# l90lpa/fv3-jedi-linearmodel

Measured on AMD Instinct MI355X. Metric: column-updates/s per TL+AD dyn step, higher is better.
Workload: dtype f64; 1 GPU; C192L127 hydrostatic TL+AD, six cube faces dealt over 1 GPU(s) (6 per rank), table-driven exchange (221184 columns per GPU), k_split=2 n_split=6 dt=450s nq=4, hord mt/vt/tm/dp/tr=2/2/2/2/2 (sponge: 1/1/1/1 below level 9), kord=17, nord=1; columns_per_gpu=221184

## Files before the change

fv3_jedi_linearmodel_amd/csrc/dycore.h:

```cpp
#pragma once
#include "../../include/fv3lm.h"
#include "stages.h"
#include "column.h"
#include "exchange.h"
#include "nh.h"
#include "nh_ad.h"
#include "tpfused.h"
#include "tpad.h"
#include "tp2.h"
#include "dampt.h"
#include "dext.h"
#include "a2b.h"
#include "d2a2c.h"
#include "del6.h"
#include <functional>
#include <map>
#include <memory>
#include <set>
#include <string>
#include <vector>

namespace fv3 {

#ifdef FV3LM_HOST_EMUL
inline void* dev_alloc(size_t n) { void* p = std::calloc(n ? n : 1, 1); return p; }
inline void dev_free(void* p) { std::free(p); }
inline void dev_zero(Exec&, void* p, size_t n) { std::memset(p, 0, n); }
inline void dev_copy(Exec&, void* d, const void* s, size_t n) { std::memcpy(d, s, n); }
inline void h2d(Exec&, void* d, const void* s, size_t n) { std::memcpy(d, s, n); }
inline void d2h(Exec&, void* d, const void* s, size_t n) { std::memcpy(d, s, n); }
inline void dev_sync(Exec&) {}
#else
#define HIPCHK(x) do { hipError_t e_ = (x); if (e_ != hipSuccess) { char b_[320]; std::snprintf(b_, sizeof b_, "HIP error '%s' at %s:%d (%s)", hipGetErrorString(e_), __FILE__, __LINE__, #x); set_sticky(b_); } } while (0)
inline void* dev_alloc(size_t n) {
  void* p = nullptr;
  if (!sticky_error().empty()) return nullptr;
  const hipError_t e = hipMalloc(&p, n ? n : 8);
  if (e != hipSuccess) { char b_[200]; std::snprintf(b_, sizeof b_, "hipMalloc of %zu bytes failed: %s", n, hipGetErrorString(e)); set_sticky(b_); (void)hipGetLastError(); return nullptr; }
  HIPCHK(hipMemset(p, 0, n ? n : 8));
  return p;
}
inline void dev_free(void* p) { if (p) (void)hipFree(p); }
__global__ void __launch_bounds__(256) k_zero16(double2* p, size_t n2) {
  const size_t stride = (size_t)gridDim.x * 256;
  for (size_t i = (size_t)blockIdx.x * 256 + threadIdx.x; i < n2; i += stride) p[i] = make_double2(0., 0.);
}
inline void dev_zero(Exec& ex, void* p, size_t n) {
  if (n >= ((size_t)1 << 20) && ((uintptr_t)p & 7) == 0) {
    char* q = (char*)p;
    if ((uintptr_t)q & 15) { HIPCHK(hipMemsetAsync(q, 0, 8, ex.stream)); q += 8; n -= 8; }
    const size_t n2 = n / 16, want = (n2 + 255) / 256;
    hipLaunchKernelGGL(k_zero16, dim3((unsigned)(want < 8192 ? want : 8192)), dim3(256), 0, ex.stream, (double2*)q, n2);
    if (n & 15) HIPCHK(hipMemsetAsync(q + n2 * 16, 0, n & 15, ex.stream));
    return;
  }
  HIPCHK(hipMemsetAsync(p, 0, n, ex.stream));
}
inline void dev_copy(Exec& ex, void* d, const void* s, size_t n) { HIPCHK(hipMemcpyAsync(d, s, n, hipMemcpyDeviceToDevice, ex.stream)); }
inline void h2d(Exec& ex, void* d, const void* s, size_t n) { HIPCHK(hipMemcpyAsync(d, s, n, hipMemcpyHostToDevice, ex.stream)); HIPCHK(hipStreamSynchronize(ex.stream)); }
inline void d2h(Exec& ex, void* d, const void* s, size_t n) { HIPCHK(hipMemcpyAsync(d, s, n, hipMemcpyDeviceToHost, ex.stream)); HIPCHK(hipStreamSynchronize(ex.stream)); }
inline void dev_sync(Exec& ex) { HIPCHK(hipStreamSynchronize(ex.stream)); }
#endif

struct Arena {
  double* t = nullptr; double* p = nullptr; size_t cap = 0, used = 0;
  void measure() { cap = (size_t)1 << 56; t = p = (double*)(uintptr_t)4096; used = 0; }
  void init(size_t ndoubles) { cap = ndoubles; t = (double*)dev_alloc(cap * 8); p = (double*)dev_alloc(cap * 8); used = 0; }
  void destroy() { dev_free(t); dev_free(p); t = p = nullptr; }
  Fld take(size_t n, int nk) {
    if (used + n > cap) { set_sticky("internal sizing error: field arena overflow"); Fld f; f.t = t; f.p = p; f.nk = nk; return f; }
    Fld f; f.t = t + used; f.p = p + used; f.nk = nk; used += n; return f;
  }
};

struct CkSet {
  struct Item { std::string name; double* p; size_t n, off; };
  std::string name; std::vector<Item> items; size_t stride = 0; int nrec = 0; double* buf = nullptr;
  void add(const std::string& nm, double* p, size_t ndoubles) { items.push_back(Item{nm, p, ndoubles, stride}); stride += ndoubles; }
  void add(const std::string& nm, const Fld& f, size_t plane) { add(nm, f.t, (size_t)f.nk * plane); }
  void alloc(const char* nm, int nrec_) {
    name = nm; buf = nrec_ > 0 ? (double*)dev_alloc(stride * nrec_ * 8) : nullptr; nrec = buf ? nrec_ : 0;
    if (std::getenv("FV3LM_VERBOSE")) std::fprintf(stderr, "fv3lm: checkpoint set %s: %d records, %zu bytes\n", nm, nrec, stride * nrec * 8);
  }
  void destroy() { dev_free(buf); buf = nullptr; nrec = 0; }
  int item(const char* nm) const {
    for (int n = 0; n < (int)items.size(); ++n) if (items[(size_t)n].name == nm) return n;
    set_sticky("internal error: checkpoint set " + name + " has no item " + nm); return -1;
  }
  size_t bytes(int item) const { return items[(size_t)item].n * 8; }
  double* at(int rec, int item) const {
    if (buf && rec >= 0 && rec < nrec && item >= 0 && item < (int)items.size()) return buf + (size_t)rec * stride + items[(size_t)item].off;
    set_sticky("internal error: checkpoint set " + name + ": record " + std::to_string(rec) + " item " + std::to_string(item) + " out of range"); return nullptr;
  }
  void save(Exec& ex, int rec, int item) const { if (double* q_ = at(rec, item)) dev_copy(ex, q_, items[(size_t)item].p, bytes(item)); }
  void restore(Exec& ex, int rec, int item, double* to = nullptr) const {
    if (const double* q_ = at(rec, item)) dev_copy(ex, to ? to : items[(size_t)item].p, q_, bytes(item));
  }
  void save(Exec& ex, int rec) const { for (int n = 0; n < (int)items.size(); ++n) save(ex, rec, n); }
  void restore(Exec& ex, int rec) const { for (int n = 0; n < (int)items.size(); ++n) restore(ex, rec, n); }
  void redirect(Exec& ex, int rec, int item, const double* from) const { if (double* q_ = at(rec, item)) ex.redirect_t(from, q_); }
};

typedef fv3lm_options Options;

inline bool resolve_level(const Options& o, int k, int npz, LevelParams& lp) {
  int hord_m = o.hord_mt, hord_t = o.hord_tm, hord_v = o.hord_vt, hord_p = o.hord_dp;
  int nord_k = o.nord, nord_v = (2 > o.nord) ? o.nord : 2;
  double d2_divg = (0.20 > o.d2_bg) ? o.d2_bg : 0.20;
  double damp_vt = o.do_vort_damp ? o.vtdm4 : 0.;
  int nord_w = nord_v, nord_t = nord_v;
  double damp_w = damp_vt, damp_t = damp_vt, d_con_k = o.d_con;
  if (npz == 1 || o.n_sponge < 0) {
    d2_divg = o.d2_bg;
  } else if (k == 1) {
    nord_k = 0;
    if (0.01 < o.d2_bg) d2_divg = (o.d2_bg < o.d2_bg_k1) ? o.d2_bg_k1 : o.d2_bg;
    else if (0.01 < o.d2_bg_k1) d2_divg = o.d2_bg_k1;
    else d2_divg = 0.01;
    nord_w = 0; damp_w = d2_divg;
    if (o.do_vort_damp) { nord_v = 0; damp_vt = 0.5 * d2_divg; }
    d_con_k = 0.;
  } else {
    const int max1 = (2 < o.n_sponge - 1) ? o.n_sponge - 1 : 2;
    if (k == max1 && o.d2_bg_k2 > 0.01) {
      nord_k = 0; d2_divg = (o.d2_bg < o.d2_bg_k2) ? o.d2_bg_k2 : o.d2_bg;
      nord_w = 0; damp_w = d2_divg;
      if (o.do_vort_damp) { nord_v = 0; damp_vt = 0.5 * d2_divg; }
      d_con_k = 0.;
    } else {
      const int max2 = (3 < o.n_sponge) ? o.n_sponge : 3;
      if (k == max2 && o.d2_bg_k2 > 0.05) {
        nord_k = 0; d2_divg = (o.d2_bg < 0.2 * o.d2_bg_k2) ? 0.2 * o.d2_bg_k2 : o.d2_bg;
        nord_w = 0; damp_w = d2_divg; d_con_k = 0.;
      }
    }
  }
  int hmp = o.hord_mt_pert, htp = o.hord_tm_pert, hvp = o.hord_vt_pert, hpp = o.hord_dp_pert;
  int nord_k_pert = o.nord_pert;
  int nord_v_pert = (2 > o.nord_pert) ? o.nord_pert : 2;
  double damp_vt_pert = o.do_vort_damp_pert ? o.vtdm4_pert : 0.;
  double d2_divg_pert = (0.20 > o.d2_bg_pert) ? o.d2_bg_pert : 0.20;
  const int nord_t_pert = nord_v_pert; const double damp_t_pert = damp_vt_pert;
  if (k <= o.n_sponge_pert) {
    nord_k_pert = 0;
    if (k <= o.n_sponge_pert - 1) {
      if (o.hord_ks_traj) { hord_m = o.hord_mt_ks_traj; hord_t = o.hord_tm_ks_traj; hord_v = o.hord_vt_ks_traj; hord_p = o.hord_dp_ks_traj; }
      if (o.hord_ks_pert) { hmp = o.hord_mt_ks_pert; htp = o.hord_tm_ks_pert; hvp = o.hord_vt_ks_pert; hpp = o.hord_dp_ks_pert; }
    }
    const double kfac = (k == 1) ? o.d2_bg_k1_pert : (k == 2) ? o.d2_bg_k2_pert : o.d2_bg_ks_pert;
    double d2p;
    if (0.01 < o.d2_bg_pert) d2p = (o.d2_bg_pert < kfac) ? kfac : o.d2_bg_pert;
    else if (0.01 < kfac) d2p = kfac;
    else d2p = 0.01;
    d2_divg_pert = d2p;
    if (o.do_vort_damp_pert) { nord_v_pert = 0; damp_vt_pert = 0.5 * d2p; }
  }
  lp.hord_mt = hmp; lp.hord_vt = hvp; lp.hord_tm = htp; lp.hord_dp = hpp; lp.hord_tr = o.hord_tr_pert;
  lp.hord_tm_g = o.hord_tm_pert;
  lp.hord_mt_t = hord_m; lp.hord_vt_t = hord_v; lp.hord_tm_t = hord_t; lp.hord_dp_t = hord_p; lp.hord_tr_t = o.hord_tr; lp.hord_tm_g_t = o.hord_tm;
  lp.nord = nord_k; lp.nord_v = nord_v; lp.nord_w = nord_w; lp.nord_t = nord_t; lp.nord_v_pert = nord_v_pert;
  lp.d2_divg = d2_divg; lp.damp_vt = damp_vt; lp.damp_w = damp_w; lp.damp_t = damp_t; lp.d_con = d_con_k;
  lp.damp_vt_pert = damp_vt_pert;
  lp.split_damp = o.split_damp ? 1 : 0; lp.nord_t_pert = nord_t_pert; lp.damp_t_pert = damp_t_pert;
  lp.dddmp = o.dddmp; lp.d4_bg = o.d4_bg;
  if (o.split_damp) { lp.nord_p = nord_k_pert; lp.d2_divg_p = d2_divg_pert; lp.dddmp_p = o.dddmp_pert; lp.d4_bg_p = o.d4_bg_pert; }
  else { lp.nord_p = nord_k; lp.d2_divg_p = d2_divg; lp.dddmp_p = o.dddmp; lp.d4_bg_p = o.d4_bg; }
// ... 845 lines not shown
  { const char* e = std::getenv("FV3LM_NH_TAPE"); a.use_tape = (e && e[0] == '1') ? 1 : 0; }
  a.dt = dt_; a.akap = opt.akap; a.ptop = opt.ptop; a.rdgas = opt.rdgas; a.grav = opt.grav; a.a_imp = opt.a_imp; a.p_fac = opt.p_fac; a.scale_z = opt.scale_z;
  return a;
}
inline void Dycore::add_col(Program& P, const char* group, int kind, const NhColArgs& a, Rect r, Rect skip, int when) {
  Dycore* self = this;
  static const char* tags[][3] = {{"riem_c.nl", "riem_c.tl", "riem_c.ad"}, {"riem3.nl", "riem3.tl", "riem3.ad"}, {"edge_profile.nl", "edge_profile.tl", "edge_profile.ad"},
                                  {"zh_init.nl", "zh_init.tl", "zh_init.ad"}, {"p_ring.nl", "p_ring.tl", "p_ring.ad"},
                                  {"remap_field_nh.nl", "remap_field_nh.tl", "remap_field_nh.ad"}, {"remap_press_nh.nl", "remap_press_nh.tl", "remap_press_nh.ad"},
                                  {"remap_w_nh.nl", "remap_w_nh.tl", "remap_w_nh.ad"}, {"remap_field_nh_lim.nl", "remap_field_nh_lim.tl", "remap_field_nh_lim.ad"},
                                  {"remap_w_nh_lim.nl", "remap_w_nh_lim.tl", "remap_w_nh_lim.ad"}};
  Op op{group, [self, kind, a, r, skip, when](Exec& e, int mode) {
    if (when == 2 && !self->last_acoustic) return;
    NhColArgs b = a; b.last_call = (when == 3 ? self->remap_last : self->last_acoustic) ? 1 : 0;
    run_nh_col(e, mode, b, kind, r, skip, tags[kind][mode]);
  }};
  const int nin = kind == NHC_RIEM_C ? 4 : kind == NHC_RIEM3 ? 4 : kind == NHC_EDGE ? 2 : kind == NHC_RING ? 1 : 0;
  const int nout = kind == NHC_RIEM_C ? 2 : kind == NHC_RIEM3 ? 9 : kind == NHC_EDGE ? 2 : kind == NHC_RING ? 1 : 0;
  for (int n = 0; n < nin; ++n) op.ad_in.push_back(a.f[n].p);
  for (int n = 0; n < nout; ++n) { op.ad_out.push_back(a.f[nin + n].p); op.ad_out_rect.push_back(r); }
  P.push_back(op);
}
inline bool Dycore::nh_overflow() {
  if (!nh) return false;
  int flag = 0; d2h(ex, &flag, nh_tape.overflow, 4);
  return flag != 0;
}

inline void Dycore::build_acoustic() {
  const int is = g.is(), ie = g.ie(), js = g.js(), je = g.je(), isd = g.isd(), ied = g.ied(), jsd = g.jsd(), jed = g.jed(), npz = g.npz;
  const double dt = bdt / double(n_split) / double(k_split), dt2 = 0.5 * dt;
  Program& P = acoustic;
  Fld u = S("u", npz), v = S("v", npz), delp = S("delp", npz), pt = S("pt", npz);
  Fld u_o = W("u_o", npz), v_o = W("v_o", npz), delp_o = W("delp_o", npz), pt_o = W("pt_o", npz);
  Fld mfx = S("mfx", npz), mfy = S("mfy", npz), cx = S("cx", npz), cy = S("cy", npz);
  Fld pe = S("pe", npz + 1), peln = S("peln", npz + 1), pk = S("pk", npz + 1), pkz = S("pkz", npz);
  st_in = {"u", "v", "delp", "pt"}; st_out = {"u_o", "v_o", "delp_o", "pt_o"};
  Fld w{}, delz{}, zh{}, w_o{}, delz_o{}, zh_o{};
  if (nh) {
    w = S("w", npz); delz = S("delz", npz); zh = S("zh", npz + 1);
    w_o = W("w_o", npz); delz_o = W("delz_o", npz); zh_o = W("zh_o", npz + 1);
    for (const char* n_ : {"w", "delz", "zh"}) st_in.push_back(n_);
    for (const char* n_ : {"w_o", "delz_o", "zh_o"}) st_out.push_back(n_);
  }
  Fld utmp = W("utmp", npz), vtmp = W("vtmp", npz), ua = W("ua", npz), va = W("va", npz);
  const bool d2c_fused = switch_on("FV3LM_D2A2C_FUSED");
  D2a2cArgs d2c; d2c.u = u; d2c.v = v; d2c.ua = ua; d2c.va = va; d2c.utmp = utmp; d2c.vtmp = vtmp; d2c.dt2 = dt2; d2c.nk = npz; d2c.face = g.face ? 1 : 0;
  d2c.ru = d2c.rv = d2c.ra = Rect{1, 0, 1, 0};
  const size_t d2c_n0 = P.size();
  { CswInterpAD s; s.in[0] = u; s.in[1] = v; s.out[0] = utmp; s.out[1] = vtmp; s.out[2] = ua; s.out[3] = va;
    s.orect[0] = R(isd, ied, js - 1, je + 1); s.orect[1] = R(is - 1, ie + 1, jsd, jed);
    s.orect[2] = s.orect[3] = R(is - 1, ie + 1, js - 1, je + 1);
    if (g.face) {
      const int il = is == 1 ? isd : is - 1, ih = ie == g.nx ? ied : ie + 1, jl = js == 1 ? jsd : js - 1, jh = je == g.ny ? jed : je + 1;
      s.orect[0] = R(isd, ied, jl, jh); s.orect[1] = R(il, ih, jsd, jed); s.orect[2] = s.orect[3] = R(il, ih, jl, jh);
    }
    s.k1 = npz;
    if (!d2c_fused) add_face(P, "c_sw", s, 3);
    else {
      const Rect both[2] = {s.orect[0], s.orect[1]};
      d2c.rtmp = rect_union(both, 2);
      d2c.ra = g.face ? isect(s.orect[2], R(4, g.nx - 3, 4, g.nx - 3)) : s.orect[2];
      if (is_empty(d2c.ra)) d2c.ra = Rect{1, 0, 1, 0};
      if (g.face) add_multi(P, "c_sw", face_strips(s, 3));
    } }
  Fld uc0 = W("uc0", npz), utf = W("utf", npz), vc0 = W("vc0", npz), vtf = W("vtf", npz);
  d2c.uc0 = uc0; d2c.utf = utf; d2c.vc0 = vc0; d2c.vtf = vtf;
  const Fld none{};
  { CswInterpC_<false> s; s.in[0] = utmp; s.in[1] = vtmp; s.in[2] = u; s.in[3] = v; s.out[0] = uc0; s.out[1] = utf; s.out[2] = vc0; s.out[3] = vtf;
    s.dt2 = dt2; s.k1 = npz;
    if (!g.face) {
      s.orect[0] = s.orect[1] = R(is - 1, ie + 2, js - 1, je + 1); s.orect[2] = s.orect[3] = R(is - 1, ie + 1, js - 1, je + 2);
      if (!d2c_fused) add(P, "c_sw", s);
      else { d2c.ru = s.orect[0]; d2c.rv = s.orect[2]; }
    } else {
      const int npx = g.nx + 1, npy = g.ny + 1;
      const Rect ur = R(is - 1, ie + 2, js - 1, je + 1), vr = R(is - 1, ie + 1, js - 1, je + 2);
      s.orect[0] = s.orect[1] = isect(ur, R(3, npx - 2, ur.j0, ur.j1)); s.orect[2] = s.orect[3] = isect(vr, R(vr.i0, vr.i1, 3, npy - 2));
      const bool b0 = !is_empty(s.orect[0]), b2 = !is_empty(s.orect[2]);
      if (b0 && !b2) s.orect[2] = s.orect[3] = empty_in(s.orect[0]);
      if (b2 && !b0) s.orect[0] = s.orect[1] = empty_in(s.orect[2]);
      CswInterpC_<true> e; for (int n = 0; n < 4; ++n) { e.in[n] = s.in[n]; e.out[n] = s.out[n]; }
      e.in[4] = ua; e.in[5] = va; e.dt2 = dt2; e.k1 = npz;
      std::vector<CswInterpC_<true>> ev;
      for (int m = 0; m < 4; ++m) {
        const Rect r = m == 0 ? isect(ur, R(ur.i0, 2, ur.j0, ur.j1)) : m == 1 ? isect(ur, R(npx - 1, ur.i1, ur.j0, ur.j1)) : m == 2 ? isect(vr, R(vr.i0, vr.i1, vr.j0, 2)) : isect(vr, R(vr.i0, vr.i1, npy - 1, vr.j1));
        if (is_empty(r)) continue;
        e.orect[0] = e.orect[1] = m < 2 ? r : empty_in(r); e.orect[2] = e.orect[3] = m < 2 ? empty_in(r) : r; ev.push_back(e);
      }
      add_multi(P, "c_sw", ev);
      if (!d2c_fused) { if (b0 || b2) add(P, "c_sw", s); }
      else { if (b0) d2c.ru = s.orect[0]; if (b2) d2c.rv = s.orect[2]; }
    } }
  if (d2c_fused && !is_empty(d2c.all())) {
    d2c.clear_tmp = (g.face && utmp.p && vtmp.p) ? 1 : 0;
    TiledAd ad; ad.in = {u.p, v.p}; ad.in_slot = {0, 1};
    ad.out = {uc0.p, utf.p, vc0.p, vtf.p, ua.p, va.p};
    ad.out_rect = {d2c.ru, d2c.ru, d2c.rv, d2c.rv, d2c.ra, d2c.ra};
    if (d2c.clear_tmp) ad.store = {utmp.p, vtmp.p};
    const size_t d2c_n1 = P.size();
    add_tiled(P, "c_sw", "D2a2c", std::make_shared<D2a2cArgs>(d2c), run_d2a2c, 7u, ad);
    beside_bulk(P, d2c_n0, d2c_n1);
  }
  Fld divgd = W("divgd", npz);
  if (opt.nord > 0) {
    CswDivgD s; s.in[0] = u; s.in[1] = v; s.in[2] = ua; s.in[3] = va; s.out[0] = divgd; s.orect[0] = R(is, ie + 1, js, je + 1); s.k1 = npz;
    add_face(P, "c_sw", s, 1);
  }
  Fld delpc = W("delpc", npz), ptc = W("ptc", npz);
  { CswTransportD s; s.in[0] = delp; s.in[1] = pt; s.in[2] = utf; s.in[3] = vtf; s.out[0] = delpc; s.out[1] = ptc;
    s.orect[0] = s.orect[1] = R(is - 1, ie + 1, js - 1, je + 1); s.k1 = npz; add_face(P, "c_sw", s, 1); }
  const bool dext = dext_on();
  Fld dx_wk{}, dx_dvt{}, divg2{}, dx_w{};
  if (dext) {
    dx_wk = W("dext_wk", npz);
    A2bOrd2D s; s.in[0] = delp; s.out[0] = dx_wk; s.orect[0] = R(is, ie + 1, js, je + 1); s.k1 = npz; add_face(P, "d_ext", s, 1);
  }
  Fld wc{};
  if (nh) {
    wc = W("wc", npz);
    CswTransportWD s; s.in[0] = delp; s.in[1] = w; s.in[2] = utf; s.in[3] = vtf; s.in[4] = delpc; s.out[0] = wc;
    s.orect[0] = R(is - 1, ie + 1, js - 1, je + 1); s.k1 = npz; add_face(P, "c_sw", s, 1);
  }
  Fld ke_c = W("ke_c", npz), vort_c = W("vort_c", npz);
  { CswKeVortD s; s.in[0] = ua; s.in[1] = va; s.in[2] = uc0; s.in[3] = vc0; s.in[4] = g.face ? u : none; s.in[5] = g.face ? v : none; s.out[0] = ke_c; s.out[1] = vort_c;
    s.orect[0] = R(is - 1, ie + 1, js - 1, je + 1); s.orect[1] = R(is, ie + 1, js, je + 1); s.dt2 = dt2; s.k1 = npz; add_face(P, "c_sw", s, 1); }
  Fld uc1 = W("uc1", npz), vc1 = W("vc1", npz);
  { CswUpdateD s; s.in[0] = uc0; s.in[1] = vc0; s.in[2] = u; s.in[3] = v; s.in[4] = vort_c; s.in[5] = ke_c; s.out[0] = uc1; s.out[1] = vc1;
    s.orect[0] = R(is, ie + 1, js, je); s.orect[1] = R(is, ie, js, je + 1); s.dt2 = dt2; s.k1 = npz; add_face(P, "c_sw", s, 1); }
  Fld pe_c = W("pe_c", npz + 1), peln_c = W("peln_c", npz + 1), pkc = W("pkc", npz + 1), gz = W("gz", npz + 1);
  Fld uc = W("uc", npz), vc = W("vc", npz);
  if (nh) {
    Fld gz_a = W("gz_a", npz + 1);
    Fld xfz = W("xfz", npz + 1), yfz = W("yfz", npz + 1);
    { DzFluxC s; s.in[0] = utf; s.in[1] = vtf; s.out[0] = xfz; s.out[1] = yfz; s.orect[0] = R(is - 1, ie + 2, js - 1, je + 1);
      s.orect[1] = R(is - 1, ie + 1, js - 1, je + 2); s.k1 = npz + 1; add(P, "update_dz_c", s); }
    { UpdateDzCD s; s.in[0] = zh; s.in[1] = xfz; s.in[2] = yfz; s.out[0] = gz_a; s.orect[0] = R(is - 1, ie + 1, js - 1, je + 1); s.k1 = npz + 1;
      add_face(P, "update_dz_c", s, 1); }
    { NhColArgs a = nh_args(dt2); a.f[0] = gz_a; a.f[1] = wc; a.f[2] = ptc; a.f[3] = delpc; a.f[4] = gz; a.f[5] = pkc;
      add_col(P, "riem_c", NHC_RIEM_C, a, R(is - 1, ie + 1, js - 1, je + 1)); }
    PGradCNh s; s.in[0] = pkc; s.in[1] = gz; s.in[2] = uc1; s.in[3] = vc1; s.in[4] = delpc; s.out[0] = uc; s.out[1] = vc;
    s.orect[0] = R(is, ie + 1, js, je); s.orect[1] = R(is, ie, js, je + 1); s.dt2 = dt2; s.k1 = npz; add(P, "p_grad_c", s);
  } else {
  { GeopkArgs a; a.g = g; a.R = R(is - 1, ie + 1, js - 1, je + 1); a.delp = delpc; a.pt = ptc; a.pe = pe_c; a.peln = peln_c; a.pk = pkc;
    a.gz = gz; a.pkz = Fld{}; a.hs = hs_dev; a.ptop = opt.ptop; a.akap = opt.akap; a.cp_air = opt.cp_air; a.cg = 1;
    Op op{"geopk_c", [a](Exec& e, int mode) { run_geopk(e, mode, a); }};
    op.ad_in = {a.delp.p, a.pt.p}; op.ad_out = {a.pe.p, a.peln.p, a.pk.p, a.gz.p}; op.ad_out_rect.assign(4, a.R);
    P.push_back(op); }
  { PGradC s; s.in[0] = pkc; s.in[1] = gz; s.in[2] = uc1; s.in[3] = vc1; s.out[0] = uc; s.out[1] = vc;
    s.orect[0] = R(is, ie + 1, js, je); s.orect[1] = R(is, ie, js, je + 1); s.dt2 = dt2; s.k1 = npz; add(P, "p_grad_c", s); }
  }
  add_halo(P, "halo_uc", H_CVEC, uc, vc);
  Fld ut = W("ut", npz), crx = W("crx", npz), xfx = W("xfx", npz), vt = W("vt", npz), cry = W("cry", npz), yfx = W("yfx", npz);
  if (!g.face) {
    DswWinds s; s.in[0] = uc; s.in[1] = vc; s.out[0] = ut; s.out[1] = crx; s.out[2] = xfx; s.out[3] = vt; s.out[4] = cry; s.out[5] = yfx;
    s.orect[0] = R(is - 1, ie + 2, jsd, jed); s.orect[1] = s.orect[2] = R(is, ie + 1, jsd, jed);
    s.orect[3] = R(isd, ied, js - 1, je + 2); s.orect[4] = s.orect[5] = R(isd, ied, js, je + 1); s.dt = dt; s.k1 = npz; add(P, "d_sw", s);
  } else {
    Fld ut_a = W("ut_a", npz), vt_a = W("vt_a", npz);
    { DswWindsAD s; s.in[0] = uc; s.in[1] = vc; s.out[0] = ut_a; s.out[1] = vt_a; s.orect[0] = R(is - 1, ie + 2, jsd, jed); s.orect[1] = R(isd, ied, js - 1, je + 2);
      s.dt = dt; s.k1 = npz; add_face(P, "d_sw", s, 1); }
    Fld ut_e = W("ut_e", npz), vt_e = W("vt_e", npz);
    const int npx = g.nx + 1, npy = g.ny + 1;
    DswWindsE se; se.in[0] = ut_a; se.in[1] = vt_a; se.in[2] = uc; se.in[3] = vc; se.out[0] = ut_e; se.out[1] = vt_e; se.k1 = npz;
    std::vector<DswWindsE> sv;
    for (int e = 0; e < 4; ++e) {
      const Rect r = e == 0 ? isect(R(is - 1, ie + 2, jsd, jed), R(is - 1, ie + 2, 0, 1)) : e == 1 ? isect(R(is - 1, ie + 2, jsd, jed), R(is - 1, ie + 2, npy - 1, npy))
                   : e == 2 ? isect(R(isd, ied, js - 1, je + 2), R(0, 1, js - 1, je + 2)) : isect(R(isd, ied, js - 1, je + 2), R(npx - 1, npx, js - 1, je + 2));
      if (is_empty(r)) continue;
      se.orect[e < 2 ? 0 : 1] = r; se.orect[e < 2 ? 1 : 0] = empty_in(r); sv.push_back(se);
    }
    add_multi(P, "d_sw", sv);
    DswWindsCD s; s.in[0] = ut_a; s.in[1] = vt_a; s.in[2] = ut_e; s.in[3] = vt_e; s.out[0] = ut; s.out[1] = crx; s.out[2] = xfx; s.out[3] = vt; s.out[4] = cry; s.out[5] = yfx;
    s.orect[0] = R(is - 1, ie + 2, jsd, jed); s.orect[1] = s.orect[2] = R(is, ie + 1, jsd, jed);
    s.orect[3] = R(isd, ied, js - 1, je + 2); s.orect[4] = s.orect[5] = R(isd, ied, js, je + 1); s.dt = dt; s.k1 = npz; add_face(P, "d_sw", s, 1);
  }
  Fld rax = W("ra_x", npz), ray = W("ra_y", npz);
  { DswRa s; s.in[0] = xfx; s.in[1] = yfx; s.out[0] = rax; s.out[1] = ray; s.orect[0] = R(is, ie, jsd, jed); s.orect[1] = R(isd, ied, js, je);
    s.k1 = npz; add(P, "d_sw", s); }
  Fld fx = W("fx", npz), fy = W("fy", npz), gx = W("gx", npz), gy = W("gy", npz);
  const Fld acc4[4] = {cx, cy, mfx, mfy};
  const bool tpf_on = switch_on("FV3LM_TP_FUSED");
  build_tp(P, "d_sw", "tpd", delp, crx, cry, xfx, yfx, rax, ray, xfx, yfx, Fld{}, HORD_DP, DAMP_V, false, fx, fy, 0, tpf_on ? acc4 : nullptr);
  { const size_t n0 = P.size();
    add_accum(P, "d_sw", cx, crx, R(is, ie + 1, jsd, jed)); add_accum(P, "d_sw", mfx, fx, R(is, ie + 1, js, je));
    add_accum(P, "d_sw", cy, cry, R(isd, ied, js, je + 1)); add_accum(P, "d_sw", mfy, fy, R(is, ie, js, je + 1));
    if (tpf_on) for (size_t n = n0; n < P.size(); ++n) P[n].modes = 1u << MODE_AD; }
  Fld w_m{}, dw{}, gxw{}, gyw{};
  if (nh) {
    Fld d6w = W("del6_w", npz); dw = W("dw", npz); gxw = W("gxw", npz); gyw = W("gyw", npz); w_m = W("w_m", npz);
    bool n2 = false;
    for (int k = 0; k < npz; ++k) n2 = n2 || Del6BD::on(lev_host[k], 0);
    const int r1 = n2 ? 2 : 1;
    const size_t n_d6 = P.size();
    { Del6AD s; s.in[0] = w; s.out[0] = d6w; s.orect[0] = R(is - r1, ie + r1, js - r1, je + r1); s.k1 = npz; add_face(P, "d_sw", s, 1); }
    if (!n2) { DswDw s; s.in[0] = w; s.in[1] = d6w; s.out[0] = dw; s.orect[0] = R(is, ie, js, je); s.k1 = npz; add(P, "d_sw", s); }
    else {
      Fld d6bw = W("del6b_w", npz);
      { Del6BD s; s.in[0] = d6w; s.out[0] = d6bw; s.orect[0] = R(is - 1, ie + 1, js - 1, je + 1); s.k1 = npz; s.sel = 0; add_face(P, "d_sw", s, 1); }
      DswDwT<true> s; s.in[0] = w; s.in[1] = d6w; s.in[2] = d6bw; s.out[0] = dw; s.orect[0] = R(is, ie, js, je); s.k1 = npz; add(P, "d_sw", s);
      const unsigned mt = del6_tiled_modes();
      for (size_t n = n_d6; n < P.size(); ++n) P[n].modes = 7u & ~mt;
      if (mt) add_del6(P, "d_sw", w, dw, npz, 0, mt);
    }
    build_tp(P, "d_sw", "tpw", w, crx, cry, xfx, yfx, rax, ray, fx, fy, Fld{}, HORD_VT, DAMP_NONE, false, gxw, gyw);
  }
  build_tp(P, "d_sw", "tpt", pt, crx, cry, xfx, yfx, rax, ray, fx, fy, delp, HORD_TM, DAMP_T, true, gx, gy);
  { DswUpdateDp s; s.in[0] = delp; s.in[1] = pt; s.in[2] = fx; s.in[3] = fy; s.in[4] = gx; s.in[5] = gy; s.out[0] = delp_o; s.out[1] = pt_o;
    s.orect[0] = s.orect[1] = R(is, ie, js, je); s.k1 = npz; add(P, "d_sw", s); }
  if (nh) {
    DswUpdateW s; s.in[0] = w; s.in[1] = delp; s.in[2] = delp_o; s.in[3] = gxw; s.in[4] = gyw; s.in[5] = dw; s.out[0] = w_m;
    s.orect[0] = R(is, ie, js, je); s.k1 = npz; add(P, "d_sw", s);
  }
  Fld vb = W("vb", npz), ub = W("ub", npz), ke = W("ke", npz);
  { DswKeWindsD s; s.in[0] = uc; s.in[1] = vc; s.in[2] = g.face ? ut : none; s.in[3] = g.face ? vt : none; s.out[0] = vb; s.out[1] = ub; s.orect[0] = s.orect[1] = R(is, ie + 1, js, je + 1); s.dt = dt;
    s.k1 = npz; add_face(P, "d_sw", s, 1); }
  { bool split_mt = false;
    for (int k = 0; k < npz; ++k) split_mt = split_mt || level_split(lev_host[k], HORD_MT);
    auto ke_stage = [&](auto s) { s.in[0] = vb; s.in[1] = ub; s.in[2] = u; s.in[3] = v; s.in[4] = g.face ? ut : none; s.in[5] = g.face ? vt : none; s.dt = dt; s.out[0] = ke; s.orect[0] = R(is, ie + 1, js, je + 1); s.k1 = npz; add_face(P, "d_sw", s, 3); };
    if (split_mt) ke_stage(DswKeSD{}); else ke_stage(DswKeD{}); }
  Fld wk = W("wk", npz), vorta = W("vort_abs", npz);
  { DswVort s; s.in[0] = u; s.in[1] = v; s.out[0] = wk; s.out[1] = vorta; s.orect[0] = s.orect[1] = R(isd, ied, jsd, jed); s.k1 = npz; add(P, "d_sw", s); }
  Fld da = W("dd_a", npz), db = W("dd_b", npz), dc = W("dd_c", npz), vortb = W("vort_b", npz), ke2 = W("ke2", npz);
  if (opt.nord > 0) add_halo_async(P, "halo_divgd", H_CORNER, divgd);
  { DdAD s; s.in[0] = divgd; s.in[1] = u; s.in[2] = v; s.in[3] = ua; s.in[4] = va; s.in[5] = g.face ? uc : none; s.in[6] = g.face ? vc : none; s.out[0] = da; s.out[1] = db;
    s.orect[0] = R(is - 1, ie + 1, js, je + 1); s.orect[1] = R(is, ie + 1, js - 1, je + 1); s.k1 = npz; add_face(P, "d_sw", s, 1); }
  { DdBD s; s.in[0] = da; s.in[1] = db; s.out[0] = dc; s.orect[0] = R(is, ie + 1, js, je + 1); s.k1 = npz; add_face(P, "d_sw", s, 1); }
  build_a2b(P, "d_sw", "a2bw", wk, vortb, npz);
  { DdC s; s.in[0] = ke; s.in[1] = dc; s.in[2] = divgd; s.in[3] = vortb; s.out[0] = ke2; s.orect[0] = R(is, ie + 1, js, je + 1);
    s.dt = dt; s.k1 = npz; add(P, "d_sw", s); }
  { bool need = false; int max_nord = 0;
    for (int k = 0; k < npz; ++k) { const LevelParams& l = lev_host[k]; max_nord = std::max(max_nord, l.nord);
      need = need || (l.split_damp && (l.nord != l.nord_p || l.d2_divg != l.d2_divg_p || l.dddmp != l.dddmp_p || l.d4_bg != l.d4_bg_p)); }
    if (need) {
      Fld s1 = max_nord >= 1 ? W("ddt_s1", npz) : Fld{}, s2 = max_nord >= 2 ? W("ddt_s2", npz) : Fld{};
      if (dext) dx_dvt = W("dext_dvt", npz);
      const Fld dvt = dx_dvt;
      Dycore* self = this;
      Op op{"d_sw", [self, u, v, ua, va, uc, vc, divgd, vortb, ke, ke2, s1, s2, dt, max_nord, dvt](Exec& e, int) {
        DampTArgs a; a.g = self->g; a.m = self->ctx.m; a.lev = self->lev_dev;
        a.u = e.sh(u).t; a.v = e.sh(v).t; a.ua = e.sh(ua).t; a.va = e.sh(va).t; a.uc = e.sh(uc).t; a.vc = e.sh(vc).t;
        a.divgd = e.sh(divgd).t; a.vortb = e.sh(vortb).t; a.ke = e.sh(ke).t; a.ke2 = e.sh(ke2).t; a.s1 = e.sh(s1).t; a.s2 = e.sh(s2).t; a.dt = dt;
        a.dvt = e.sh(dvt).t;
        run_damp_t(e, a, max_nord);
      }};
      op.modes = (1u << MODE_NL) | (1u << MODE_TL); op.name = "DampT";
      P.push_back(op);
    } }
  if (dext) {
    divg2 = W("divg2", 1); dx_w = W("dext_w", 1);
    const Fld wkc = dx_wk, dvt = dx_dvt, d2 = divg2, ws = dx_w, dgf = opt.nord > 0 ? divgd : Fld{};
    Dycore* self = this;
    Op op{"d_ext", [self, wkc, dc, dgf, dvt, d2, ws](Exec& e, int mode) {
      DextArgs a{}; a.g = self->g; a.lev = self->lev_dev; a.cfac = self->d_ext * self->ctx.m.da_min_c;
      a.wk = e.sh(wkc); a.dc = e.sh(dc); a.dg = e.sh(dgf); a.dvt = e.sh(dvt).t; a.d2 = e.sh(d2); a.ws = e.sh(ws);
      run_dext_col(e, mode, a);
    }};
    op.ad_in = {wkc.p, dc.p}; if (dgf.p) op.ad_in.push_back(dgf.p);
    op.ad_store = op.ad_in;
    op.ad_out = {d2.p}; op.ad_out_rect = {R(is, ie + 1, js, je + 1)};
    op.name = "DextCol";
    P.push_back(op);
  }
  Fld fxv = W("fxv", npz), fyv = W("fyv", npz);
  build_tp(P, "d_sw", "tpv", vorta, crx, cry, xfx, yfx, rax, ray, xfx, yfx, Fld{}, HORD_VT, DAMP_NONE, false, fxv, fyv);
  Fld d6 = W("del6_d2", npz);
  { Del6AD s; s.in[0] = wk; s.out[0] = d6; s.orect[0] = R(is - 1, ie + 1, js - 1, je + 1); s.k1 = npz; add_face(P, "d_sw", s, 1); }
  Fld u_m = W("u_m", npz), v_m = W("v_m", npz);
  { bool n2 = false;
    for (int k = 0; k < npz; ++k) n2 = n2 || Del6BD::on(lev_host[k], 1);
    auto uv_stage = [&](auto s) { s.in[0] = u; s.in[1] = v; s.in[2] = ke2; s.in[3] = fxv; s.in[4] = fyv; s.in[5] = wk; s.in[6] = d6; s.out[0] = u_m; s.out[1] = v_m;
      s.orect[0] = R(is, ie, js, je + 1); s.orect[1] = R(is, ie + 1, js, je); s.k1 = npz; return s; };
    if (!n2) add(P, "d_sw", uv_stage(DswUpdateUV{}));
    else {
      Fld l1 = W("d6t_a", npz), l2 = W("d6t_b", npz);
      Dycore* self = this;
      Op op{"d_sw", [self, wk, l1, l2](Exec& e, int) {
        const Geom& g_ = self->g;
        LapTArgs a{g_, self->ctx.m, self->lev_dev, e.sh(wk).t, e.sh(l1).t, 1};
        for_points(e, Rect{g_.is() - 2, g_.ie() + 2, g_.js() - 2, g_.je() + 2}, g_.ntile * g_.npz, LapTPass{a}, "LapT.1", 0.);
        a.src = e.sh(l1).t; a.dst = e.sh(l2).t; a.pass = 2;
        for_points(e, Rect{g_.is() - 1, g_.ie() + 1, g_.js() - 1, g_.je() + 1}, g_.ntile * g_.npz, LapTPass{a}, "LapT.2", 0.);
      }};
      op.modes = (1u << MODE_NL) | (1u << MODE_TL); op.name = "LapT";
      P.push_back(op);
      auto s2 = uv_stage(DswUpdateUVT<true>{}); s2.in[7] = l2; add(P, "d_sw", s2);
    } }
  add_halo_async(P, "halo_dp", H_CELL, delp_o); add_halo_async(P, "halo_dp", H_CELL, pt_o);
  if (nh) {
    Fld crx_e = W("crx_e", npz + 1), xfx_e = W("xfx_e", npz + 1), cry_e = W("cry_e", npz + 1), yfx_e = W("yfx_e", npz + 1);
    { NhColArgs a = nh_args(dt); a.f[0] = crx; a.f[1] = xfx; a.f[2] = crx_e; a.f[3] = xfx_e; add_col(P, "update_dz_d", NHC_EDGE, a, R(is, ie + 1, jsd, jed)); }
    { NhColArgs a = nh_args(dt); a.f[0] = cry; a.f[1] = yfx; a.f[2] = cry_e; a.f[3] = yfx_e; add_col(P, "update_dz_d", NHC_EDGE, a, R(isd, ied, js, je + 1)); }
    Fld rax_e = W("ra_x_e", npz + 1), ray_e = W("ra_y_e", npz + 1);
    { DswRa s; s.in[0] = xfx_e; s.in[1] = yfx_e; s.out[0] = rax_e; s.out[1] = ray_e; s.orect[0] = R(is, ie, jsd, jed); s.orect[1] = R(isd, ied, js, je);
      s.k1 = npz + 1; add(P, "update_dz_d", s); }
    Fld fxz = W("fxz", npz + 1), fyz = W("fyz", npz + 1), d6z = W("del6_z", npz + 1), zh_a = W("zh_a", npz + 1);
    build_tp(P, "update_dz_d", "tpz", zh, crx_e, cry_e, xfx_e, yfx_e, rax_e, ray_e, xfx_e, yfx_e, Fld{}, HORD_TM_G, DAMP_NONE, false, fxz, fyz, npz + 1);
    bool n2z = false;
    for (int k = 0; k <= npz; ++k) n2z = n2z || Del6BD::on(lev_host[k], 1);
    const int r1 = n2z ? 2 : 1;
    const size_t n_d6z = P.size();
    { Del6AD s; s.in[0] = zh; s.out[0] = d6z; s.orect[0] = R(is - r1, ie + r1, js - r1, je + r1); s.k1 = npz + 1; add_face(P, "update_dz_d", s, 1); }
    auto dz_stage = [&](auto s) { s.in[0] = zh; s.in[1] = d6z; s.in[2] = fxz; s.in[3] = fyz; s.in[4] = rax_e; s.in[5] = ray_e; s.out[0] = zh_a;
      s.orect[0] = R(is, ie, js, je); s.k1 = npz + 1; return s; };
    if (!n2z) add(P, "update_dz_d", dz_stage(UpdateDzD{}));
    else {
      Fld d6bz = W("del6b_z", npz + 1);
      { Del6BD s; s.in[0] = d6z; s.out[0] = d6bz; s.orect[0] = R(is - 1, ie + 1, js - 1, je + 1); s.k1 = npz + 1; s.sel = 1; add_face(P, "update_dz_d", s, 1); }
      auto s2 = dz_stage(UpdateDzDT<true>{}); s2.in[6] = d6bz; add(P, "update_dz_d", s2);
      const unsigned mt = del6_tiled_modes();
      for (size_t n = n_d6z; n < P.size(); ++n) P[n].modes = 7u & ~mt;
      if (mt) {
        Fld dz6 = W("del6_dz", npz + 1);
        add_del6(P, "update_dz_d", zh, dz6, npz + 1, 1, mt);
        auto s3 = dz_stage(UpdateDzDF{}); s3.in[1] = dz6; add(P, "update_dz_d", s3); P.back().modes = mt;
      }
    }
    Fld ppe = W("ppe", npz + 1), pk3 = W("pk3", npz + 1);
    { NhColArgs a = nh_args(dt); a.f[0] = zh_a; a.f[1] = w_m; a.f[2] = pt_o; a.f[3] = delp_o; a.f[4] = w_o; a.f[5] = delz_o; a.f[6] = zh_o; a.f[7] = ppe;
      a.f[8] = pk3; a.f[9] = pe; a.f[10] = peln; a.f[11] = pk; a.f[12] = S("ws", 1); add_col(P, "riem3", NHC_RIEM3, a, R(is, ie, js, je)); }
    add_halo(P, "halo_zh", H_CELL, zh_o); add_halo(P, "halo_zh", H_CELL, ppe);
    { NhColArgs a = nh_args(dt); a.f[0] = delp_o; a.f[1] = pe; a.what = 1;
      add_col(P, "p_ring", NHC_RING, a, R(is - 1, ie + 1, js - 1, je + 1), R(is, ie, js, je), 2); }
    { NhColArgs a = nh_args(dt); a.f[0] = delp_o; a.f[1] = pk3; a.what = 0;
      add_col(P, "p_ring", NHC_RING, a, R(is - 2, ie + 2, js - 2, je + 2), R(is, ie, js, je)); }
    Fld pp_b = W("pp_b", npz + 1), pk_b = W("pk3_b", npz + 1), zh_b = W("zh_b", npz + 1), dp_b = W("dp_b", npz);
    build_a2b(P, "nh_p_grad", "a2bpp", ppe, pp_b, npz + 1);
    build_a2b(P, "nh_p_grad", "a2bpk", pk3, pk_b, npz + 1);
// ... 121 lines not shown
```

Baseline: 192,100 column-updates/s.

## Add fused tiled LDS kernel for d_sw wind/Courant computation with bulk/edge split

Introduces a tiled kernel that stages uc/vc into LDS per 64x16 tile and computes ut, vt, Courant numbers and fluxes in one pass, with a hand-written adjoint that accumulates into uc/vc from LDS-staged intermediates. On cube faces, the interior bulk goes through the fused kernel while the edge-corrected path runs only on boundary strips. This targets redundant global reloads of neighbouring winds and several separate launches. It adds complexity in rect bookkeeping and clearing of auxiliary adjoint buffers, and is gated behind an environment switch.

```diff
diff --git a/fv3_jedi_linearmodel_amd/csrc/dswwinds.h b/fv3_jedi_linearmodel_amd/csrc/dswwinds.h
--- /dev/null
+++ b/fv3_jedi_linearmodel_amd/csrc/dswwinds.h
@@ -0,0 +1,250 @@
+#pragma once
+#include "stages.h"
+#include "tiled.h"
+
+namespace fv3 {
+
+struct DswWindsArgs {
+  Fld uc, vc;
+  Fld ut, crx, xfx, vt, cry, yfx;
+  Fld ut_a, vt_a, ut_e, vt_e;
+  Rect rut, rcx, rvt, rcy;
+  Rect rclr{1, 0, 1, 0};
+  double dt = 0.;
+  int nk = 0;
+  int clear = 0;
+  unsigned wmask = 0;
+  Rect wrect{1, 0, 1, 0};
+  Rect all() const { return rect_join(rut, rvt); }
+};
+FV3LM_LINK void run_dsw_winds(Exec& ex, int mode, const DswWindsArgs& a0, const Ctx& c);
+
+inline double dsw_winds_bytes(const DswWindsArgs& a, const Geom& g, int mode) {
+  const Rect q = a.all();
+  const double cells = double(q.i1 - q.i0 + 1) * double(q.j1 - q.j0 + 1) * g.ntile * a.nk;
+  return 8. * cells * (mode == MODE_NL ? 8. : mode == MODE_TL ? 16. : 12.);
+}
+}
+
+#if !defined(FV3LM_SPLIT_BUILD) || defined(FV3LM_IMPL_DSWWINDS)
+namespace fv3 {
+#ifndef FV3LM_DSWWINDS_THREADS_NL
+#define FV3LM_DSWWINDS_THREADS_NL 128
+#endif
+#ifndef FV3LM_DSWWINDS_THREADS_TL
+#define FV3LM_DSWWINDS_THREADS_TL 512
+#endif
+#ifndef FV3LM_DSWWINDS_THREADS_AD
+#define FV3LM_DSWWINDS_THREADS_AD 256
+#endif
+constexpr int DSW_W = 64, DSW_H = 16;
+constexpr int DSW_QW = DSW_W + 1, DSW_QH = DSW_H + 1;
+constexpr int DSW_NQ = DSW_QW * DSW_QH, DSW_NB = DSW_W * DSW_H, DSW_NT = 2 * DSW_NQ, DSW_NT_AD = 2 * DSW_NQ + 2 * DSW_NB;
+#ifdef FV3LM_HOST_EMUL
+#define DSW_UNROLL
+#else
+#define DSW_UNROLL _Pragma("unroll")
+#endif
+enum { W_CU, W_RU, W_XW, W_X0, W_DY, W_S3, W_S1, W_CV, W_RV, W_YS, W_Y0, W_DX, W_S4, W_S2, W_N };
+HD int dsw_clamp(int m, int lo, int hi) { return m <= lo ? lo + 1 : m > hi ? hi : m; }
+HD int dsw_plane(int m, int lo, int hi) { return m < lo ? lo : m > hi ? hi : m; }
+
+template <class T, int NTH>
+DEV void dsw_winds_block(const DswWindsArgs& a, const Ctx& c, const Rect& Qr, int tile, int k, int bx, int by, double* lds, int tid) {
+  typedef TpfIO<T> IO;
+  const Geom& g = c.g;
+  const TileBlk B = tile_blk(Qr, bx, by, DSW_W, DSW_H);
+  const int I0 = B.I0, I1 = B.I1, J0 = B.J0, J1 = B.J1;
+  const int ilo = g.isd(), ihi = g.ied() + 1, jlo = g.jsd(), jhi = g.jed() + 1;
+  double* const U = lds; double* const V = U + DSW_NQ;
+  {
+    constexpr int E = (DSW_NQ + NTH - 1) / NTH;
+    auto ci = [&](int i) { return dsw_plane(i, ilo, ihi); };
+    auto cj = [&](int j) { return dsw_plane(j, jlo, jhi); };
+    T ru[E], rv[E];
+    DSW_UNROLL
+    for (int s = 0; s < E; ++s) {
+      const int e = (tid + s * NTH < DSW_NQ) ? tid + s * NTH : DSW_NQ - 1, x = e % DSW_QW, r = e / DSW_QW;
+      ru[s] = IO::ld(a.uc, fld_at(g, a.uc, tile, k, ci(I0 + x), cj(J0 - 1 + r)));
+      rv[s] = IO::ld(a.vc, fld_at(g, a.vc, tile, k, ci(I0 - 1 + x), cj(J0 + r)));
+    }
+    DSW_UNROLL
+    for (int s = 0; s < E; ++s) {
+      const int e = tid + s * NTH;
+      if (e < DSW_NQ) { IO::lset(U, DSW_NT, e, ru[s]); IO::lset(V, DSW_NT, e, rv[s]); }
+    }
+  }
+  constexpr int E3 = (DSW_NB + NTH - 1) / NTH;
+  double mt[E3][W_N];
+  DSW_UNROLL
+  for (int s = 0; s < E3; ++s) {
+    const int e = (tid + s * NTH < DSW_NB) ? tid + s * NTH : DSW_NB - 1;
+    const int i = (I0 + e % DSW_W < I1) ? I0 + e % DSW_W : I1, j = (J0 + e / DSW_W < J1) ? J0 + e / DSW_W : J1;
+    const int iu = dsw_clamp(i, ilo, ihi), jv = dsw_clamp(j, jlo, jhi);
+    double* const m = mt[s];
+    m[W_CU] = MET(cosa_u, iu, j); m[W_RU] = MET(rsin_u, iu, j); m[W_XW] = MET(rdxa, iu - 1, j); m[W_X0] = MET(rdxa, iu, j);
+    m[W_DY] = MET(dy, iu, j); m[W_S3] = SSG(3, iu - 1, j); m[W_S1] = SSG(1, iu, j);
+    m[W_CV] = MET(cosa_v, i, jv); m[W_RV] = MET(rsin_v, i, jv); m[W_YS] = MET(rdya, i, jv - 1); m[W_Y0] = MET(rdya, i, jv);
+    m[W_DX] = MET(dx, i, jv); m[W_S4] = SSG(4, i, jv - 1); m[W_S2] = SSG(2, i, jv);
+  }
+  TPF_SYNC();
+  DSW_UNROLL
+  for (int s = 0; s < E3; ++s) {
+    const int e = tid + s * NTH;
+    if (e >= DSW_NB) continue;
+    const int x = e % DSW_W, r = e / DSW_W, i = I0 + x, j = J0 + r;
+    if (i > I1 || j > J1) continue;
+    const double* const mm = mt[s];
+    auto uc = [&](int ii, int jj) -> T { return IO::lget(U, DSW_NT, (jj - (J0 - 1)) * DSW_QW + (ii - I0)); };
+    auto vc = [&](int ii, int jj) -> T { return IO::lget(V, DSW_NT, (jj - J0) * DSW_QW + (ii - (I0 - 1))); };
+    if (a.rut.has(i, j)) {
+      const T ut = (uc(i, j) - 0.25 * mm[W_CU] * (vc(i - 1, j) + vc(i, j) + vc(i - 1, j + 1) + vc(i, j + 1))) * mm[W_RU];
+      const size_t m = fld_at(g, a.ut, tile, k, i, j);
+      IO::st(a.ut, m, ut);
+      if (a.rcx.has(i, j)) {
+        const T xx = a.dt * ut;
+        T crx, xfx;
+        if (val(xx) > 0.) { crx = xx * mm[W_XW]; xfx = mm[W_DY] * xx * mm[W_S3]; }
+        else              { crx = xx * mm[W_X0]; xfx = mm[W_DY] * xx * mm[W_S1]; }
+        IO::st(a.crx, m, crx); IO::st(a.xfx, m, xfx);
+      }
+    }
+    if (a.rvt.has(i, j)) {
+      const T vt = (vc(i, j) - 0.25 * mm[W_CV] * (uc(i, j - 1) + uc(i + 1, j - 1) + uc(i, j) + uc(i + 1, j))) * mm[W_RV];
+      const size_t m = fld_at(g, a.vt, tile, k, i, j);
+      IO::st(a.vt, m, vt);
+      if (a.rcy.has(i, j)) {
+        const T yy = a.dt * vt;
+        T cry, yfx;
+        if (val(yy) > 0.) { cry = yy * mm[W_YS]; yfx = mm[W_DX] * yy * mm[W_S4]; }
+        else              { cry = yy * mm[W_Y0]; yfx = mm[W_DX] * yy * mm[W_S2]; }
+        IO::st(a.cry, m, cry); IO::st(a.yfx, m, yfx);
+      }
+    }
+  }
+}
+
+template <int NTH>
+DEV void dsw_winds_ad_block(const DswWindsArgs& a, const Ctx& c, const Rect& Qr, int tile, int k, int bx, int by, double* lds, int tid) {
+  const Geom& g = c.g;
+  const TileBlk B = tile_blk(Qr, bx, by, DSW_W, DSW_H);
+  const int I0 = B.I0, I1 = B.I1, J0 = B.J0, J1 = B.J1;
+  const int ilo = g.isd(), ihi = g.ied() + 1, jlo = g.jsd(), jhi = g.jed() + 1;
+  double* const HU = lds; double* const HV = HU + DSW_NQ; double* const GU = HV + DSW_NQ; double* const GV = GU + DSW_NB;
+  constexpr int E1 = (DSW_NQ + NTH - 1) / NTH;
+  {
+    double q[E1][11];
+    DSW_UNROLL
+    for (int s = 0; s < E1; ++s) {
+      const int e = (tid + s * NTH < DSW_NQ) ? tid + s * NTH : DSW_NQ - 1;
+      const int i = dsw_clamp(I0 + e % DSW_QW, ilo, ihi), j = dsw_plane(J0 - 1 + e / DSW_QW, jlo, jhi);
+      const size_t m = fld_at(g, a.ut, tile, k, i, j);
+      q[s][0] = a.ut.t[m]; q[s][1] = a.ut.p[m]; q[s][2] = a.crx.p[m]; q[s][3] = a.xfx.p[m];
+      q[s][4] = MET(rdxa, i - 1, j); q[s][5] = MET(rdxa, i, j); q[s][6] = MET(dy, i, j); q[s][7] = SSG(3, i - 1, j); q[s][8] = SSG(1, i, j);
+      q[s][9] = MET(rsin_u, i, j); q[s][10] = MET(cosa_u, i, j);
+    }
+    DSW_UNROLL
+    for (int s = 0; s < E1; ++s) {
+      const int e = tid + s * NTH;
+      if (e >= DSW_NQ) continue;
+      const int x = e % DSW_QW, r = e / DSW_QW, i = I0 + x, j = J0 - 1 + r;
+      double gu = 0.;
+      if (a.rut.has(i, j)) {
+        double tot = q[s][1];
+        if (a.rcx.has(i, j)) {
+          const bool pos = a.dt * q[s][0] > 0.;
+          tot += a.dt * ((pos ? q[s][4] : q[s][5]) * q[s][2] + q[s][6] * (pos ? q[s][7] : q[s][8]) * q[s][3]);
+        }
+        gu = q[s][9] * tot;
+      }
+      HU[e] = q[s][10] * gu;
+      if (x < DSW_W && r >= 1) GU[(r - 1) * DSW_W + x] = gu;
+    }
+  }
+  {
+    double q[E1][11];
+    DSW_UNROLL
+    for (int s = 0; s < E1; ++s) {
+      const int e = (tid + s * NTH < DSW_NQ) ? tid + s * NTH : DSW_NQ - 1;
+      const int i = dsw_plane(I0 - 1 + e % DSW_QW, ilo, ihi), j = dsw_clamp(J0 + e / DSW_QW, jlo, jhi);
+      const size_t m = fld_at(g, a.vt, tile, k, i, j);
+      q[s][0] = a.vt.t[m]; q[s][1] = a.vt.p[m]; q[s][2] = a.cry.p[m]; q[s][3] = a.yfx.p[m];
+      q[s][4] = MET(rdya, i, j - 1); q[s][5] = MET(rdya, i, j); q[s][6] = MET(dx, i, j); q[s][7] = SSG(4, i, j - 1); q[s][8] = SSG(2, i, j);
+      q[s][9] = MET(rsin_v, i, j); q[s][10] = MET(cosa_v, i, j);
+    }
+    DSW_UNROLL
+    for (int s = 0; s < E1; ++s) {
+      const int e = tid + s * NTH;
+      if (e >= DSW_NQ) continue;
+      const int x = e % DSW_QW, r = e / DSW_QW, i = I0 - 1 + x, j = J0 + r;
+      double gv = 0.;
+      if (a.rvt.has(i, j)) {
+        double tot = q[s][1];
+        if (a.rcy.has(i, j)) {
+          const bool pos = a.dt * q[s][0] > 0.;
+          tot += a.dt * ((pos ? q[s][4] : q[s][5]) * q[s][2] + q[s][6] * (pos ? q[s][7] : q[s][8]) * q[s][3]);
+        }
+        gv = q[s][9] * tot;
+      }
+      HV[e] = q[s][10] * gv;
+      if (x >= 1 && r < DSW_H) GV[r * DSW_W + (x - 1)] = gv;
+    }
+  }
+  constexpr int E3 = (DSW_NB + NTH - 1) / NTH;
+  const bool acc_u = a.uc.p && !(a.wmask & 1u), acc_v = a.vc.p && !(a.wmask & 2u);
+  double q[E3][2];
+  DSW_UNROLL
+  for (int s = 0; s < E3; ++s) {
+    const int e = (tid + s * NTH < DSW_NB) ? tid + s * NTH : DSW_NB - 1;
+    const int i = (I0 + e % DSW_W < I1) ? I0 + e % DSW_W : I1, j = (J0 + e / DSW_W < J1) ? J0 + e / DSW_W : J1;
+    const size_t m = fld_at(g, a.uc, tile, k, i, j);
+    q[s][0] = acc_u ? a.uc.p[m] : 0.; q[s][1] = acc_v ? a.vc.p[m] : 0.;
+  }
+  TPF_SYNC();
+  DSW_UNROLL
+  for (int s = 0; s < E3; ++s) {
+    const int e = tid + s * NTH;
+    if (e >= DSW_NB) continue;
+    const int x = e % DSW_W, r = e / DSW_W, i = I0 + x, j = J0 + r;
+    if (i > I1 || j > J1) continue;
+    const double* const hv = HV + r * DSW_QW + x;
+    const double* const hu = HU + r * DSW_QW + x;
+    const double au = GU[e] - 0.25 * (hv[0] + hv[1] + hv[DSW_QW] + hv[DSW_QW + 1]);
+    const double av = GV[e] - 0.25 * (hu[0] + hu[1] + hu[DSW_QW] + hu[DSW_QW + 1]);
+    const size_t m = fld_at(g, a.uc, tile, k, i, j);
+    if (a.uc.p) a.uc.p[m] = q[s][0] + au;
+    if (a.vc.p) a.vc.p[m] = q[s][1] + av;
+    if (a.clear && a.rclr.has(i, j) && !(i >= 3 && i <= g.nx - 2 && j >= 3 && j <= g.ny - 2)) { a.ut_a.p[m] = 0.; a.vt_a.p[m] = 0.; a.ut_e.p[m] = 0.; a.vt_e.p[m] = 0.; }
+  }
+}
+
+template <class T, int N> struct DswWindsFwd {
+  typedef DswWindsArgs Args; static constexpr int NTH = N; static constexpr size_t LDS_BYTES = (size_t)DSW_NT * 8 * TpfIO<T>::NC;
+  DEV static void block(const Args& a, const Ctx& c, const Rect& Qr, int tile, int k, int bx, int by, double* lds, int tid) { dsw_winds_block<T, N>(a, c, Qr, tile, k, bx, by, lds, tid); }
+};
+template <int N> struct DswWindsAd {
+  typedef DswWindsArgs Args; static constexpr int NTH = N; static constexpr size_t LDS_BYTES = (size_t)DSW_NT_AD * 8;
+  DEV static void block(const Args& a, const Ctx& c, const Rect& Qr, int tile, int k, int bx, int by, double* lds, int tid) { dsw_winds_ad_block<N>(a, c, Qr, tile, k, bx, by, lds, tid); }
+};
+
+FV3LM_LINK void run_dsw_winds(Exec& ex, int mode, const DswWindsArgs& a0, const Ctx& c) {
+  DswWindsArgs a = a0;
+  for (Fld* f : {&a.uc, &a.vc, &a.ut, &a.crx, &a.xfx, &a.vt, &a.cry, &a.yfx, &a.ut_a, &a.vt_a, &a.ut_e, &a.vt_e}) *f = ex.sh(*f);
+  if (ex.no_wmask) a.wmask = 0;
+  if (!a.ut_a.p || !a.vt_a.p || !a.ut_e.p || !a.vt_e.p) a.clear = 0;
+  if (mode == MODE_AD && !a.uc.p && !a.vc.p && !a.clear) return;
+  Rect Qr = a.all();
+  if (mode == MODE_AD) {
+    Qr.i0 -= 1; Qr.i1 += 1; Qr.j0 -= 1; Qr.j1 += 1;
+    if (a.clear) Qr = rect_join(Qr, a.rclr);
+    Qr = ad_launch_rect(Qr, a.wmask != 0, a.wrect, c.g);
+  }
+  const int nbx = tiled_blocks(Qr.i0, Qr.i1, DSW_W), nby = tiled_blocks(Qr.j0, Qr.j1, DSW_H);
+  const double bytes = dsw_winds_bytes(a, c.g, mode);
+  if (mode == MODE_TL) run_tiled<DswWindsFwd<Dual, tiled_nth(FV3LM_DSWWINDS_THREADS_TL)>>(ex, "DswWindsF", mode_tag(mode), bytes, Qr, nbx, nby, a, c);
+  else if (mode == MODE_NL) run_tiled<DswWindsFwd<double, tiled_nth(FV3LM_DSWWINDS_THREADS_NL)>>(ex, "DswWindsF", mode_tag(mode), bytes, Qr, nbx, nby, a, c);
+  else run_tiled<DswWindsAd<tiled_nth(FV3LM_DSWWINDS_THREADS_AD)>>(ex, "DswWindsF", mode_tag(mode), bytes, Qr, nbx, nby, a, c);
+}
+
+}
+#endif
diff --git a/fv3_jedi_linearmodel_amd/csrc/dycore.h b/fv3_jedi_linearmodel_amd/csrc/dycore.h
--- a/fv3_jedi_linearmodel_amd/csrc/dycore.h
+++ b/fv3_jedi_linearmodel_amd/csrc/dycore.h
@@ -12,6 +12,7 @@
 #include "dext.h"
 #include "a2b.h"
 #include "d2a2c.h"
+#include "dswwinds.h"
 #include "del6.h"
 #include <functional>
 #include <map>
@@ -1163,14 +1164,33 @@
   }
   add_halo(P, "halo_uc", H_CVEC, uc, vc);
   Fld ut = W("ut", npz), crx = W("crx", npz), xfx = W("xfx", npz), vt = W("vt", npz), cry = W("cry", npz), yfx = W("yfx", npz);
+  const bool dsw_fused = switch_on("FV3LM_DSW_WINDS_FUSED");
+  DswWindsArgs dw_; dw_.uc = uc; dw_.vc = vc; dw_.ut = ut; dw_.crx = crx; dw_.xfx = xfx; dw_.vt = vt; dw_.cry = cry; dw_.yfx = yfx; dw_.dt = dt; dw_.nk = npz;
+  dw_.rut = R(is - 1, ie + 2, jsd, jed); dw_.rcx = R(is, ie + 1, jsd, jed); dw_.rvt = R(isd, ied, js - 1, je + 2); dw_.rcy = R(isd, ied, js, je + 1);
+  auto add_dsw_fused = [&]() {
+    TiledAd ad; ad.in = {uc.p, vc.p}; ad.in_slot = {0, 1};
+    ad.out = {ut.p, crx.p, xfx.p, vt.p, cry.p, yfx.p};
+    ad.out_rect = {dw_.rut, dw_.rcx, dw_.rcx, dw_.rvt, dw_.rcy, dw_.rcy};
+    if (dw_.clear) ad.store = {dw_.ut_a.p, dw_.vt_a.p, dw_.ut_e.p, dw_.vt_e.p};
+    add_tiled(P, "d_sw", "DswWindsF", std::make_shared<DswWindsArgs>(dw_), run_dsw_winds, 7u, ad);
+  };
   if (!g.face) {
+    if (dsw_fused) add_dsw_fused();
+    else {
     DswWinds s; s.in[0] = uc; s.in[1] = vc; s.out[0] = ut; s.out[1] = crx; s.out[2] = xfx; s.out[3] = vt; s.out[4] = cry; s.out[5] = yfx;
     s.orect[0] = R(is - 1, ie + 2, jsd, jed); s.orect[1] = s.orect[2] = R(is, ie + 1, jsd, jed);
     s.orect[3] = R(isd, ied, js - 1, je + 2); s.orect[4] = s.orect[5] = R(isd, ied, js, je + 1); s.dt = dt; s.k1 = npz; add(P, "d_sw", s);
+    }
   } else {
     Fld ut_a = W("ut_a", npz), vt_a = W("vt_a", npz);
+    const Rect bulk = R(2, g.nx - 1, 2, g.nx - 1);
+    const Rect full[4] = {dw_.rut, dw_.rcx, dw_.rvt, dw_.rcy};
+    dw_.rut = isect(full[0], bulk); dw_.rcx = isect(full[1], bulk); dw_.rvt = isect(full[2], bulk); dw_.rcy = isect(full[3], bulk);
+    const bool fuse = dsw_fused && !is_empty(dw_.rut) && !is_empty(dw_.rcx) && !is_empty(dw_.rvt) && !is_empty(dw_.rcy);
+    const size_t dsw_n0 = P.size();
     { DswWindsAD s; s.in[0] = uc; s.in[1] = vc; s.out[0] = ut_a; s.out[1] = vt_a; s.orect[0] = R(is - 1, ie + 2, jsd, jed); s.orect[1] = R(isd, ied, js - 1, je + 2);
-      s.dt = dt; s.k1 = npz; add_face(P, "d_sw", s, 1); }
+      s.dt = dt; s.k1 = npz;
+      if (!fuse) add_face(P, "d_sw", s, 1); else add_multi(P, "d_sw", face_strips(s, 2)); }
     Fld ut_e = W("ut_e", npz), vt_e = W("vt_e", npz);
     const int npx = g.nx + 1, npy = g.ny + 1;
     DswWindsE se; se.in[0] = ut_a; se.in[1] = vt_a; se.in[2] = uc; se.in[3] = vc; se.out[0] = ut_e; se.out[1] = vt_e; se.k1 = npz;
@@ -1184,7 +1204,17 @@
     add_multi(P, "d_sw", sv);
     DswWindsCD s; s.in[0] = ut_a; s.in[1] = vt_a; s.in[2] = ut_e; s.in[3] = vt_e; s.out[0] = ut; s.out[1] = crx; s.out[2] = xfx; s.out[3] = vt; s.out[4] = cry; s.out[5] = yfx;
     s.orect[0] = R(is - 1, ie + 2, jsd, jed); s.orect[1] = s.orect[2] = R(is, ie + 1, jsd, jed);
-    s.orect[3] = R(isd, ied, js - 1, je + 2); s.orect[4] = s.orect[5] = R(isd, ied, js, je + 1); s.dt = dt; s.k1 = npz; add_face(P, "d_sw", s, 1);
+    s.orect[3] = R(isd, ied, js - 1, je + 2); s.orect[4] = s.orect[5] = R(isd, ied, js, je + 1); s.dt = dt; s.k1 = npz;
+    if (!fuse) add_face(P, "d_sw", s, 1);
+    else {
+      add_multi(P, "d_sw", face_strips(s, 1));
+      dw_.ut_a = ut_a; dw_.vt_a = vt_a; dw_.ut_e = ut_e; dw_.vt_e = vt_e;
+      dw_.clear = (ut_a.p && vt_a.p && ut_e.p && vt_e.p) ? 1 : 0;
+      dw_.rclr = R(isd, ied + 1, jsd, jed + 1);
+      const size_t dsw_n1 = P.size();
+      add_dsw_fused();
+      beside_bulk(P, dsw_n0, dsw_n1);
+    }
   }
   Fld rax = W("ra_x", npz), ray = W("ra_y", npz);
   { DswRa s; s.in[0] = xfx; s.in[1] = yfx; s.out[0] = rax; s.out[1] = ray; s.orect[0] = R(is, ie, jsd, jed); s.orect[1] = R(isd, ied, js, je);
diff --git a/fv3_jedi_linearmodel_amd/csrc/tu_dswwinds.cpp b/fv3_jedi_linearmodel_amd/csrc/tu_dswwinds.cpp
--- /dev/null
+++ b/fv3_jedi_linearmodel_amd/csrc/tu_dswwinds.cpp
@@ -0,0 +1,2 @@
+#define FV3LM_IMPL_DSWWINDS
+#include "dswwinds.h"
```

Result: faster. 194,600 column-updates/s, median of 6 (+1.3%).
